# kcat/openal-soft

Measured on NVIDIA H100. Metric: voice-samples/s mixed (HRTF, bsinc24, 1024-frame updates), higher is better.
Workload: dtype f32

## Files before the change

openal-soft_b200/csrc/mixer_kernels.cuh:

```cuda
#pragma once
#include <cstdint>
#include <cuda_runtime.h>

#include "voice_structs.hpp"
#include "async_ptx.cuh"

namespace b200mix {

constexpr int kLine = 1024;
constexpr int kHrirLen = 128;
constexpr int kHist = 64;
constexpr int kEdge = 24;
constexpr int kPad = 48;
constexpr int kResBuf = kLine + 256 + kPad;
constexpr int kSrcSizeMax = kResBuf - kEdge;
constexpr int kAccumLen = kLine + kHrirLen;
constexpr float kSilence = 0.00001f;
constexpr float kEps = 1.1920929e-07f;

constexpr uint32_t kVfStatic = 1u<<2, kVfLooping = 1u<<3, kVfHrtf = 1u<<4;
constexpr uint32_t kVfFading = 1u<<8, kVfHaveBuffer = 1u<<9, kVfCoefDirty = 1u<<10;
constexpr uint32_t kUpNoBuffer = 1u<<11;
constexpr uint32_t kVfChannelMask = 0xffu<<16;

struct alignas(16) BufferRec {
    const void *data;
    uint32_t frames, type, channels, pad;
};

struct alignas(16) VoiceRec {
    uint32_t state;
    uint32_t flags;
    uint32_t buffer, resampler;
    int32_t  pos; uint32_t frac, step, loop_start;
    uint32_t loop_end; float bsinc_sf; uint32_t bsinc_m, bsinc_l;
    uint32_t bsinc_off, tgt_delay0, tgt_delay1; float tgt_gain;
    uint32_t old_delay0, old_delay1; float old_gain; uint32_t send_mask;
    uint32_t send_slot[kMaxSends]; uint32_t pad2[2];
    float prev[kPad];
    float hist[kHist];
};

struct VoiceResult { int32_t position; uint32_t position_frac, flags, buffers_done; };

struct alignas(16) FilterRec {
    float cur[2][5]; float tgt[2][5];
    float z[2][2];
    int32_t counter[2];
    uint32_t active;
    uint32_t pad[5];
};
static_assert(sizeof(FilterRec) == 128, "FilterRec layout");

struct MixParams {
    VoiceRec *voices; const BufferRec *buffers;
    float2 *hrtf_tgt; float2 *hrtf_old;
    float *dry_cur; float *dry_tgt;
    float *partial;
    VoiceResult *results;
    const float *bsinc_tab[3];
    const float *cubic_tab[2];
    uint32_t max_voices, frames, ir_pad, cd, num_sends;
    float *xscratch;
    uint32_t *sendinfo;
    const uint32_t *order;
    uint32_t num_order;
    FilterRec *filt;
    uint32_t filt_paths;
    const float *dline;
    uint4 *qhdr; const uint32_t *queue;
    uint32_t *claim;
};

constexpr uint32_t kMaxQueue = 32, kNoLoop = 0xffffffffu;

constexpr uint32_t kSiSend = 1u, kSiPlaying = 2u, kSiDeferred = 4u, kSiDirty = 8u, kSiDry = 16u,
    kSiHrtf = 32u;

__device__ __forceinline__ void group_sync(int id, int count)
{
    if(id == 1) asm volatile("bar.sync 1, %0;" :: "r"(count) : "memory");
    else asm volatile("bar.sync 2, %0;" :: "r"(count) : "memory");
}

__device__ __forceinline__ void prefetch_l2(const void *p)
{ asm volatile("prefetch.global.L2 [%0];" :: "l"(p)); }

__device__ __forceinline__ uint32_t sample_bytes(uint32_t type)
{ return type == 1u ? 2u : ((type == 0u || type >= 5u) ? 1u : (type == 4u ? 8u : 4u)); }

__device__ __forceinline__ void prefetch_span(const char *base, size_t bytes, size_t off,
    size_t len, int t, int gs)
{
    if(off >= bytes) return;
    if(off + len > bytes) len = bytes - off;
    const size_t first = off & ~size_t(127);
    for(size_t a = first + size_t(t)*128u;a < off + len;a += size_t(gs)*128u)
        prefetch_l2(base + a);
}

__device__ __forceinline__ float load_sample(const BufferRec &b, size_t idx)
{
    switch(b.type)
    {
    case 0: return (float(static_cast<const uint8_t*>(b.data)[idx]) - 128.0f) * (1.0f/128.0f);
    case 1: return float(static_cast<const int16_t*>(b.data)[idx]) * (1.0f/32768.0f);
    case 2: return float(static_cast<const int32_t*>(b.data)[idx]) * (1.0f/2147483648.0f);
    case 3: return static_cast<const float*>(b.data)[idx];
    case 4: return float(static_cast<const double*>(b.data)[idx]);
    }
    return 0.0f;
}

__device__ __forceinline__ void calc_buffer_size(uint32_t fracPos, uint32_t increment,
    uint32_t dstRemaining, uint32_t &dst, uint32_t &src)
{
    const uint32_t ext = increment <= 65536u;
    const uint64_t srcSize64 = ((uint64_t(dstRemaining - ext)*increment + fracPos) >> 16)
        + ext + kEdge;
    if(srcSize64 <= uint64_t(kSrcSizeMax)) { dst = dstRemaining; src = uint32_t(srcSize64); return; }
    const uint64_t dstSize64 = ((uint64_t(kSrcSizeMax - kEdge)<<16) - fracPos) / increment;
    if(dstSize64 < dstRemaining) { dst = uint32_t(dstSize64) & ~3u; src = kSrcSizeMax; return; }
    dst = dstRemaining; src = kSrcSizeMax;
}

__device__ __forceinline__ int32_t add_sat(int32_t a, int32_t b)
{
    long long r = (long long)a + b;
    r = r > 2147483647ll ? 2147483647ll : (r < -2147483648ll ? -2147483648ll : r);
    return int32_t(r);
}

__device__ __forceinline__ float to_float(uint8_t v) { return (float(v) - 128.0f) * (1.0f/128.0f); }
__device__ __forceinline__ float to_float(int16_t v) { return float(v) * (1.0f/32768.0f); }
__device__ __forceinline__ float to_float(int32_t v) { return float(v) * (1.0f/2147483648.0f); }
__device__ __forceinline__ float to_float(float v) { return v; }
__device__ __forceinline__ float to_float(double v) { return float(v); }
struct MulawByte { uint8_t v; };
struct AlawByte { uint8_t v; };
__device__ __forceinline__ float to_float(MulawByte b)
{
    const uint32_t u = (~uint32_t(b.v)) & 0xffu;
    const int s = int((((u & 0x0fu)<<3) + 0x84u) << ((u>>4)&7u)) - 0x84;
    return float((u & 0x80u) ? -s : s) * (1.0f/32768.0f);
}
__device__ __forceinline__ float to_float(AlawByte b)
{
    const uint32_t a = uint32_t(b.v) ^ 0x55u;
    const uint32_t e = (a>>4)&7u, m = a & 0x0fu;
    const int s = (e == 0u) ? int((m<<4) + 8u) : int(((m<<4) + 0x108u) << (e-1u));
    return float((a & 0x80u) ? s : -s) * (1.0f/32768.0f);
}

template<typename T> __device__ __forceinline__ T ld_raw(const T *p) { return __ldg(p); }
template<> __device__ __forceinline__ MulawByte ld_raw(const MulawByte *p)
{ return MulawByte{__ldg(reinterpret_cast<const uint8_t*>(p))}; }
template<> __device__ __forceinline__ AlawByte ld_raw(const AlawByte *p)
{ return AlawByte{__ldg(reinterpret_cast<const uint8_t*>(p))}; }

constexpr int kPackB = 688;
static_assert(kPackB >= (kResBuf + 8 + 1)/2 && kPackB + (kResBuf + 8 + 1)/2 <= kResBuf + 8 + 24
    && (kPackB % 32) == 16, "16-bit window copies must fit the float window's storage");

__device__ __forceinline__ float win_at(const float *win, bool packed, uint32_t k)
{
    if(!packed) return win[k];
    const uint16_t y = reinterpret_cast<const uint16_t*>(win)[k];
    return float(int(y) - 32768) * (1.0f/32768.0f);
}

struct FillArgs {
    float *dst; uint32_t count, uintPos, q0, firstRun, loopStart, loopSize, lastFrame, channels;
    bool looping, pastEnd, simpleWrap;
};

__device__ __forceinline__ void filter_clear(FilterRec &fr, int t)
{
    if(t < 10) fr.cur[t/5][t%5] = fr.tgt[t/5][t%5];
    else if(t < 14) fr.z[(t-10)>>1][(t-10)&1] = 0.0f;
    else if(t < 16) fr.counter[t-14] = 0;
}

template<typename T, int GS>
__device__ __forceinline__ void fill_window(const FillArgs &A, const T *__restrict__ src, int t)
{
    for(uint32_t k0 = t;k0 < A.count;k0 += 8u*GS)
    {
        T raw[8];
        #pragma unroll
        for(int u = 0;u < 8;++u)
        {
            uint32_t k = k0 + uint32_t(u)*GS;
            k = k < A.count ? k : A.count-1u;
            uint32_t q;
            if(!A.looping) q = min(A.uintPos + k, A.lastFrame);
            else if(k < A.firstRun) q = A.q0 + k;
            else if(A.simpleWrap) q = A.loopStart + (k - A.firstRun);
            else q = A.loopStart + (k - A.firstRun)%A.loopSize;
            raw[u] = ld_raw(src + size_t(q)*A.channels);
        }
        #pragma unroll
        for(int u = 0;u < 8;++u)
        {
            const uint32_t k = k0 + uint32_t(u)*GS;
            if(k < A.count) A.dst[k] = A.pastEnd ? 0.0f : to_float(raw[u]);
        }
    }
}

constexpr int kWinFloats = kResBuf + 8 + 24;
template<int CDR>
struct alignas(16) GroupSmem {
    static constexpr int kTabStride = kPad + 2;
    float win[kWinFloats];
    alignas(8) float tabF[32*kTabStride];
    alignas(8) float tabD[32*kTabStride];
    float x[CDR > 0 ? kLine : 1];
    float newGain[32];
    uint64_t tmaBar;
    uint32_t claimed;
};

template<int GS, int OPT, int FP>
struct alignas(16) FirSmem {
    static constexpr int kLLen = FP + OPT*GS;
    static constexpr int kOLen = FP + kHist + FP + 32;
    float2 lLR[kLLen];
    float2 oLR[kOLen];
    float x[kHist + kLine];
    float2 coefT[kHrirLen], coefO[kHrirLen];
};

__device__ __forceinline__ float2 fma2_rn(float2 a, float2 b, float2 c)
{ return make_float2(__fmaf_rn(a.x, b.x, c.x), __fmaf_rn(a.y, b.y, c.y)); }

template<int OPT, int FP>
__device__ __forceinline__ void fir_pass(float2 (&acc)[OPT], const float2 *__restrict__ in,
    const float2 *__restrict__ coef, int irpad, int t0)
{
    constexpr int JB = 8;
    for(int jb = 0;jb < irpad;jb += JB)
    {
        float2 w[OPT+JB-1];
        const float2 *p = in + FP + t0 - jb - (JB-1);
        #pragma unroll
        for(int k = 0;k < OPT+JB-1;++k) w[k] = p[k];
        #pragma unroll
        for(int jj = 0;jj < JB;++jj)
        {
            const float2 c = coef[jb+jj];
            #pragma unroll
            for(int r = 0;r < OPT;++r)
                acc[r] = fma2_rn(c, w[r - jj + (JB-1)], acc[r]);
        }
    }
}

__device__ __forceinline__ uint32_t claim_voice(const MixParams &P, uint32_t &slot, int t, int bar,
    int gs, uint32_t groups)
{
    group_sync(bar, gs);
    if(t == 0)
    {
        uint32_t oi = atomicAdd(P.claim, 1u);
        if(oi >= P.num_order && atomicAdd(P.claim + 1, 1u) == groups - 1u)
        {
            atomicExch(P.claim, 0u);
            atomicExch(P.claim + 1, 0u);
        }
        slot = oi;
    }
    group_sync(bar, gs);
    return slot;
}


__device__ __forceinline__ bool voice_early_out(const MixParams &P, VoiceRec &rec, uint32_t v,
    uint32_t vstate, uint4 h1, int t)
{
    if(vstate != 1u && vstate != 2u)
    {
        if(t == 0)
        {
            if(P.results) P.results[v] = VoiceResult{int32_t(h1.x), h1.y, 1u<<7, 0u};
            if(P.sendinfo) P.sendinfo[v] = 0u;
        }
        return true;
    }
    if(h1.z < 1u)
    {
        if(t == 0)
        {
            if(vstate == 2u) rec.state = 0u;
            if(P.sendinfo) P.sendinfo[v] = 0u;
            if(P.results)
                P.results[v] = VoiceResult{int32_t(h1.x), h1.y, (vstate == 2u) ? (1u<<7) : 1u, 0u};
        }
        return true;
    }
    return false;
}

template<int GS>
__device__ __forceinline__ void build_phase_table(const MixParams &P, float *tabF, float *tabD,
    uint32_t resampler, uint32_t increment, uint4 h2, uint4 h3, int t,
    uint32_t &m, uint32_t &tapOff, uint32_t &ms)
{
    m = 0; tapOff = 0; ms = 5;
    if(resampler >= 4u)
    {
        m = h2.z;
        tapOff = kEdge - h2.w;
        const float *tab = P.bsinc_tab[(resampler-4u)>>1] + h3.x;
        const bool full = (increment > 65536u) && (resampler & 1u);
        const float sf = __uint_as_float(h2.y);
        const uint32_t rowLen = 2u*m;
        const float *tab2 = tab + 64u*m;
        ms = m + 1u;
        for(uint32_t c = t;c < rowLen;c += GS)
        {
            float *dstc = (c < m) ? (tabF + c) : (tabD + (c - m));
            #pragma unroll 1
            for(uint32_t p0 = 0;p0 < 32u;p0 += 8u)
            {
                float a[8], b[8];
                #pragma unroll
                for(int u = 0;u < 8;++u)
                {
                    a[u] = __ldg(tab + (p0+u)*rowLen + c);
                    b[u] = full ? __ldg(tab2 + (p0+u)*rowLen + c) : 0.0f;
                }
                #pragma unroll
                for(int u = 0;u < 8;++u)
                    dstc[(p0+u)*ms] = full ? fmaf(sf, b[u], a[u]) : a[u];
            }
        }
    }
    else if(resampler >= 2u)
    {
        m = 4; tapOff = kEdge - 1; ms = 5;
        const float *tab = P.cubic_tab[resampler-2u];
        for(uint32_t e = t;e < 128u;e += GS)
        {
            const uint32_t pi = e>>2, j = e&3u;
            tabF[pi*ms + j] = tab[pi*8u + j];
            tabD[pi*ms + j] = tab[pi*8u + 4u + j];
        }
    }
}

template<int GS>
__device__ __forceinline__ void prefetch_next_voices(const MixParams &P, uint32_t oi, uint32_t groups,
    int t)
{
    const uint32_t o2 = oi + 2u*groups, o1 = oi + groups;
    const uint32_t v2 = o2 < P.num_order ? P.order[o2] : 0xffffffffu;
    const uint32_t v1 = o1 < P.num_order ? P.order[o1] : 0xffffffffu;
    if(v2 < P.max_voices && t < 5)
        prefetch_l2(reinterpret_cast<const char*>(&P.voices[v2]) + t*128);
    if(v1 < P.max_voices)
    {
        const VoiceRec &nx = P.voices[v1];
        if((nx.state == 1u || nx.state == 2u) && (nx.flags & kVfHaveBuffer) && nx.step >= 1u)
        {
            const BufferRec nb = P.buffers[nx.buffer];
            const size_t fb = size_t(sample_bytes(nb.type))*nb.channels;
            const size_t bytes = size_t(nb.frames)*fb;
            const uint32_t p0 = nx.pos < 0 ? 0u : uint32_t(nx.pos);
            const size_t need = size_t((uint64_t(P.frames)*nx.step + nx.frac) >> 16) + kPad;
            const char *base = static_cast<const char*>(nb.data);
            prefetch_span(base, bytes, size_t(p0)*fb, need*fb, t, GS);
            if((nx.flags & kVfLooping) && p0 + need > nx.loop_end && nx.loop_end > p0)
                prefetch_span(base, bytes, size_t(nx.loop_start)*fb,
                    (p0 + need - nx.loop_end)*fb, t, GS);
        }
    }
}

template<int GS>
__device__ __forceinline__ void hold_end_sample(float *srcBuffer, uint32_t srcn, int t, int bar)
{
    const uint32_t avail = srcn < uint32_t(kEdge) ? srcn : uint32_t(kEdge);
    const uint32_t tofill = srcn > uint32_t(kEdge) ? srcn : uint32_t(kEdge);
    uint32_t best = 0;
    for(uint32_t i = 1;i < avail;++i)
        if(fabsf(srcBuffer[i]) < fabsf(srcBuffer[best])) best = i;
    const float held = srcBuffer[best];
    group_sync(bar, GS);
    for(uint32_t k = best+1+t;k < tofill;k += GS) srcBuffer[k] = held;
}

template<int GS>
__device__ __forceinline__ bool stage_span_tma(float *win, uint64_t *tmaBar, uint32_t &tmaPhase,
    const BufferRec &buf, uint32_t flags, bool isQueue, bool looping, uint32_t loopStart,
    uint32_t loopEnd, uint32_t uintPos, uint32_t count, float *dst, int t, int bar)
{
    if(isQueue || buf.type != 1u || buf.channels != 1u || ((flags >> 16) & 0xffu) != 0u || count == 0u)
        return false;
    const uint32_t loopSize = looping ? (loopEnd - loopStart) : 1u;
    const uint32_t q0 = !looping ? uintPos : ((uintPos < loopEnd) ? uintPos
        : ((uintPos-loopStart)%loopSize + loopStart));
    const uint32_t run1 = looping ? min(count, loopEnd - q0) : count;
    const uint32_t run2 = count - run1;
    const bool fits = looping ? (run2 <= loopSize && loopEnd <= buf.frames)
                              : (uintPos + count <= buf.frames);
    if(!fits) return false;
    const int16_t *base = static_cast<const int16_t*>(buf.data);
    const uintptr_t a1 = reinterpret_cast<uintptr_t>(base + q0);
    const uintptr_t a2 = reinterpret_cast<uintptr_t>(base + loopStart);
    const uint32_t lead1 = uint32_t(a1 & 15u) >> 1, lead2 = uint32_t(a2 & 15u) >> 1;
    const uint32_t bytes1 = ((run1 + lead1)*2u + 15u) & ~15u;
    const uint32_t bytes2 = run2 ? (((run2 + lead2)*2u + 15u) & ~15u) : 0u;
    constexpr uint32_t kWinBytes = uint32_t(kWinFloats*sizeof(float));
    unsigned char *wbytes = reinterpret_cast<unsigned char*>(win);
    unsigned char *raw2 = wbytes + kWinBytes - bytes2;
    unsigned char *raw1 = raw2 - bytes1;
    if(t == 0)
    {
        fence_proxy_async_smem();
        mbar_expect_tx(tmaBar, bytes1 + bytes2);
        bulk_g2s(raw1, reinterpret_cast<const void*>(a1 & ~uintptr_t(15)), bytes1, tmaBar);
        if(run2)
            bulk_g2s(raw2, reinterpret_cast<const void*>(a2 & ~uintptr_t(15)), bytes2, tmaBar);
    }
    mbar_wait(tmaBar, tmaPhase);
    tmaPhase ^= 1u;
    const int16_t *r1 = reinterpret_cast<const int16_t*>(raw1) + lead1;
    const int16_t *r2 = reinterpret_cast<const int16_t*>(raw2) + lead2;
    constexpr int PERW = (kSrcSizeMax + GS - 1)/GS;
    float v[PERW];
    #pragma unroll
    for(int u = 0;u < PERW;++u)
    {
        const uint32_t k = uint32_t(t) + uint32_t(u)*GS;
        int16_t x = 0;
        if(k < count) x = k < run1 ? r1[k] : r2[k - run1];
        v[u] = to_float(x);
    }
    group_sync(bar, GS);
    #pragma unroll
    for(int u = 0;u < PERW;++u)
    {
        const uint32_t k = uint32_t(t) + uint32_t(u)*GS;
        if(k < count) dst[k] = v[u];
    }
    return true;
}

template<int GS>
__device__ __forceinline__ bool gather_span(const MixParams &P, const BufferRec &buf, uint32_t flags,
    bool isQueue, uint4 qh, const uint32_t *qitems, bool looping, uint32_t loopStart, uint32_t loopEnd,
    uint32_t uintPos, uint32_t count, float *dst, int t, int bar)
{
    uint32_t done = 0, item = qh.x ? qh.y : kNoLoop, qpos = uintPos;
    bool more = true, winInt = true;
    while(more)
    {
        BufferRec rb = buf;
        FillArgs fa;
        if(!isQueue)
        {
            const uint32_t loopSize = looping ? (loopEnd - loopStart) : 1u;
            const uint32_t q0 = !looping ? uintPos : ((uintPos < loopEnd) ? uintPos
                : ((uintPos-loopStart)%loopSize + loopStart));
            const uint32_t firstRun = looping ? (loopEnd - q0) : 0u;
            const uint32_t lastFrame = buf.frames ? buf.frames-1u : 0u;
            const bool pastEnd = !looping && !(buf.frames > uintPos);
            const bool simpleWrap = looping && count <= firstRun + loopSize;
            fa = FillArgs{dst, count, uintPos, q0, firstRun, loopStart, loopSize,
                lastFrame, buf.channels, looping, pastEnd, simpleWrap};
            done = count; more = false;
        }
        else
        {
            bool found = false;
            while(item != kNoLoop && done < count)
            {
                rb = P.buffers[qitems[item]];
                if(qpos >= rb.frames)
                {
                    qpos -= rb.frames;
                    item = (item + 1u < qh.x) ? item + 1u : qh.z;
                    continue;
                }
                found = true;
                break;
            }
            if(!found) break;
            const uint32_t run = min(count - done, rb.frames - qpos);
            fa = FillArgs{dst + done, run, qpos, qpos, 0u, 0u, 1u, rb.frames-1u,
                rb.channels, false, false, false};
            done += run; qpos = 0u;
            item = (item + 1u < qh.x) ? item + 1u : qh.z;
            more = done < count;
        }
        winInt = winInt && (rb.type <= 1u || rb.type >= 5u);
        const uint32_t ch = ((flags >> 16) & 0xffu) < rb.channels ? ((flags >> 16) & 0xffu) : 0u;
        switch(rb.type)
        {
        case 0: fill_window<uint8_t, GS>(fa, static_cast<const uint8_t*>(rb.data) + ch, t); break;
        case 1: fill_window<int16_t, GS>(fa, static_cast<const int16_t*>(rb.data) + ch, t); break;
        case 2: fill_window<int32_t, GS>(fa, static_cast<const int32_t*>(rb.data) + ch, t); break;
        case 3: fill_window<float, GS>(fa, static_cast<const float*>(rb.data) + ch, t); break;
        case 4: fill_window<double, GS>(fa, static_cast<const double*>(rb.data) + ch, t); break;
        case 5: fill_window<MulawByte, GS>(fa, static_cast<const MulawByte*>(rb.data) + ch, t); break;
        default: fill_window<AlawByte, GS>(fa, static_cast<const AlawByte*>(rb.data) + ch, t); break;
        }
    }
    if(done < count)
    {
        group_sync(bar, GS);
        const float held = done ? dst[done-1u] : 0.0f;
        for(uint32_t k = done + t;k < count;k += GS) dst[k] = held;
    }
    return winInt;
}

template<int GS>
__device__ __forceinline__ void pack_window16(float *win, uint32_t srcn, int t, int bar)
{
    constexpr int PER = (kResBuf + 8 + GS - 1)/GS;
    const uint32_t L = min(uint32_t(kEdge) + srcn + 8u, uint32_t(kResBuf + 8));
    float v[PER];
    #pragma unroll
    for(int u = 0;u < PER;++u)
    {
        const uint32_t k = uint32_t(t) + uint32_t(u)*GS;
        v[u] = k < L ? win[k] : 0.0f;
    }
    group_sync(bar, GS);
    uint16_t *pa = reinterpret_cast<uint16_t*>(win);
    uint16_t *pb = pa + 2*kPackB;
    #pragma unroll
    for(int u = 0;u < PER;++u)
    {
        const uint32_t k = uint32_t(t) + uint32_t(u)*GS;
        if(k < L)
        {
            const uint16_t y = uint16_t(__float2int_rn(v[u]*32768.0f) + 32768);
            pa[k] = y;
            if(k) pb[k-1u] = y;
        }
    }
    group_sync(bar, GS);
}

template<int GS>
__device__ __forceinline__ void resample_chunk(const float *win, const float *tabF, const float *tabD,
    float *xs, uint32_t loaded, uint32_t dstn, uint32_t increment, uint32_t fracPos,
    uint32_t resampler, uint32_t m, uint32_t tapOff, uint32_t ms, bool packedWin, int t)
{
    const float *srcBuffer = win + kEdge;
    if(increment == 65536u && fracPos == 0u)
    {
        for(uint32_t k = t;k < dstn;k += GS) xs[loaded+k] = srcBuffer[k];
    }
    else if(packedWin)
    {
        const uint32_t *wordsA = reinterpret_cast<const uint32_t*>(win);
        const uint32_t *wordsB = wordsA + kPackB;
        const float2 bias = make_float2(-8421376.0f, -8421376.0f);
        const float2 one = make_float2(1.0f, 1.0f);
        for(uint32_t k = t;k < dstn;k += 2u*GS)
        {
            const uint32_t kB = k + GS;
            const bool hasB = kB < dstn;
            const uint64_t fpA = uint64_t(k)*increment + fracPos;
            const uint64_t fpB = uint64_t(hasB ? kB : k)*increment + fracPos;
            const uint32_t fracA = uint32_t(fpA) & 0xffffu, fracB = uint32_t(fpB) & 0xffffu;
            const float pfA = float(fracA & 2047u) * (1.0f/2048.0f);
            const float pfB = float(fracB & 2047u) * (1.0f/2048.0f);
            const float *FA = tabF + (fracA>>11)*ms, *DA = tabD + (fracA>>11)*ms;
            const float *FB = tabF + (fracB>>11)*ms, *DB = tabD + (fracB>>11)*ms;
            const uint32_t posA = tapOff + uint32_t(fpA>>16), posB = tapOff + uint32_t(fpB>>16);
            const uint32_t *wA = ((posA & 1u) ? wordsB : wordsA) + (posA >> 1);
            const uint32_t *wB = ((posB & 1u) ? wordsB : wordsA) + (posB >> 1);
            const float2 pA = make_float2(pfA, pfA), pB = make_float2(pfB, pfB);
            float2 a0 = make_float2(0.0f, 0.0f), a1 = a0, b0 = a0, b1 = a0;
            for(uint32_t j = 0;j < m;j += 4)
            {
                const uint32_t wa0 = wA[(j>>1)], wa1 = wA[(j>>1)+1u];
                const uint32_t wb0 = wB[(j>>1)], wb1 = wB[(j>>1)+1u];
                const float2 sA0 = fma2_rn(make_float2(__uint_as_float(__byte_perm(wa0, 0x4B00u, 0x5410u)),
                    __uint_as_float(__byte_perm(wa0, 0x4B00u, 0x5432u))), one, bias);
                const float2 sA1 = fma2_rn(make_float2(__uint_as_float(__byte_perm(wa1, 0x4B00u, 0x5410u)),
                    __uint_as_float(__byte_perm(wa1, 0x4B00u, 0x5432u))), one, bias);
                const float2 sB0 = fma2_rn(make_float2(__uint_as_float(__byte_perm(wb0, 0x4B00u, 0x5410u)),
                    __uint_as_float(__byte_perm(wb0, 0x4B00u, 0x5432u))), one, bias);
                const float2 sB1 = fma2_rn(make_float2(__uint_as_float(__byte_perm(wb1, 0x4B00u, 0x5410u)),
                    __uint_as_float(__byte_perm(wb1, 0x4B00u, 0x5432u))), one, bias);
                const float2 cA0 = fma2_rn(pA, make_float2(DA[j+0], DA[j+1]), make_float2(FA[j+0], FA[j+1]));
                const float2 cB0 = fma2_rn(pB, make_float2(DB[j+0], DB[j+1]), make_float2(FB[j+0], FB[j+1]));
                const float2 cA1 = fma2_rn(pA, make_float2(DA[j+2], DA[j+3]), make_float2(FA[j+2], FA[j+3]));
                const float2 cB1 = fma2_rn(pB, make_float2(DB[j+2], DB[j+3]), make_float2(FB[j+2], FB[j+3]));
                a0 = fma2_rn(cA0, sA0, a0);
                b0 = fma2_rn(cB0, sB0, b0);
                a1 = fma2_rn(cA1, sA1, a1);
                b1 = fma2_rn(cB1, sB1, b1);
            }
            xs[loaded+k] = ((a0.x + a1.x) + (a0.y + a1.y)) * (1.0f/32768.0f);
            if(hasB) xs[loaded+kB] = ((b0.x + b1.x) + (b0.y + b1.y)) * (1.0f/32768.0f);
        }
    }
    else if(resampler >= 2u)
    {
        const float *vals = win + tapOff;
        for(uint32_t k = t;k < dstn;k += 2u*GS)
        {
            const uint32_t kB = k + GS;
            const bool hasB = kB < dstn;
            const uint64_t fpA = uint64_t(k)*increment + fracPos;
            const uint64_t fpB = uint64_t(hasB ? kB : k)*increment + fracPos;
            const uint32_t fracA = uint32_t(fpA) & 0xffffu, fracB = uint32_t(fpB) & 0xffffu;
            const float pfA = float(fracA & 2047u) * (1.0f/2048.0f);
            const float pfB = float(fracB & 2047u) * (1.0f/2048.0f);
            const float *FA = tabF + (fracA>>11)*ms, *DA = tabD + (fracA>>11)*ms;
            const float *FB = tabF + (fracB>>11)*ms, *DB = tabD + (fracB>>11)*ms;
            const float *svA = vals + uint32_t(fpA>>16), *svB = vals + uint32_t(fpB>>16);
            const float2 pA = make_float2(pfA, pfA), pB = make_float2(pfB, pfB);
            float2 a0 = make_float2(0.0f, 0.0f), a1 = a0, b0 = a0, b1 = a0;
            for(uint32_t j = 0;j < m;j += 4)
            {
                const float2 cA0 = fma2_rn(pA, make_float2(DA[j+0], DA[j+1]), make_float2(FA[j+0], FA[j+1]));
                const float2 cB0 = fma2_rn(pB, make_float2(DB[j+0], DB[j+1]), make_float2(FB[j+0], FB[j+1]));
                const float2 cA1 = fma2_rn(pA, make_float2(DA[j+2], DA[j+3]), make_float2(FA[j+2], FA[j+3]));
                const float2 cB1 = fma2_rn(pB, make_float2(DB[j+2], DB[j+3]), make_float2(FB[j+2], FB[j+3]));
                a0 = fma2_rn(cA0, make_float2(svA[j+0], svA[j+1]), a0);
                b0 = fma2_rn(cB0, make_float2(svB[j+0], svB[j+1]), b0);
                a1 = fma2_rn(cA1, make_float2(svA[j+2], svA[j+3]), a1);
                b1 = fma2_rn(cB1, make_float2(svB[j+2], svB[j+3]), b1);
            }
            xs[loaded+k] = (a0.x + a1.x) + (a0.y + a1.y);
            if(hasB) xs[loaded+kB] = (b0.x + b1.x) + (b0.y + b1.y);
        }
    }
    else
    {
        const float *vals = srcBuffer;
        for(uint32_t k = t;k < dstn;k += GS)
        {
            const uint64_t fp = uint64_t(k)*increment + fracPos;
            const uint32_t pos = uint32_t(fp>>16), frac = uint32_t(fp) & 0xffffu;
            if(resampler == 0u) xs[loaded+k] = vals[pos];
            else
            {
                const float a = vals[pos], b = vals[pos+1];
                xs[loaded+k] = a + (b-a)*(float(frac)*(1.0f/65536.0f));
            }
        }
    }
}

template<int GS>
__device__ __forceinline__ void advance_chunk(float *win, float *prev, bool packedWin, bool silent,
    bool playing, uint32_t n, uint32_t &loaded, uint32_t dstn, uint32_t increment, uint32_t &fracPos,
    int32_t &intPos, int t, int bar)
{
    const uint32_t loadEnd = loaded + dstn;
    if(!silent && playing && n > loaded && n <= loadEnd)
    {
        const uint32_t dstOffset = n - loaded;
        const uint32_t srcOffset = uint32_t((uint64_t(dstOffset)*increment + fracPos) >> 16);
        for(int k = t;k < kPad;k += GS) prev[k] = win_at(win, packedWin, srcOffset + uint32_t(k));
    }
    loaded = loadEnd;
    if(loaded < n)
    {
        fracPos += dstn*increment;
        const uint32_t srcOffset = fracPos >> 16;
        fracPos &= 0xffffu;
        if(silent) intPos = add_sat(intPos, int32_t(srcOffset));
        else
        {
            if(intPos < 0) intPos += int32_t(srcOffset);
            else intPos = add_sat(intPos, int32_t(srcOffset));
            float carry = 0.0f;
            if(t < kPad) carry = win_at(win, packedWin, srcOffset + uint32_t(t));
            float carry2 = 0.0f;
            if(GS < kPad && t + GS < kPad) carry2 = win_at(win, packedWin, srcOffset + uint32_t(t) + GS);
            group_sync(bar, GS);
            if(t < kPad) win[t] = carry;
            if(GS < kPad && t + GS < kPad) win[t + GS] = carry2;
        }
    }
}

template<int GS, int CDR>
__device__ __forceinline__ void park_voice(const MixParams &P, const float *xs, uint32_t v,
    uint32_t sendMask, bool defer, bool isHrtf, bool playing, bool dirty, uint32_t counter, int t)
{
    const uint32_t n = P.frames;
    const bool sends = P.num_sends && sendMask;
    const bool park = sends || defer || CDR == 0;
    if(CDR > 0 && park)
        for(uint32_t k = t;k < n;k += GS) P.xscratch[size_t(v)*kLine + k] = xs[k];
    if(t == 0)
        P.sendinfo[v] = park ? ((sends ? kSiSend : 0u)
            | (playing ? kSiPlaying : 0u) | (defer ? kSiDeferred : 0u) | (dirty ? kSiDirty : 0u)
            | ((CDR == 0 && !isHrtf) ? kSiDry : 0u) | (isHrtf ? kSiHrtf : 0u) | (counter << 8)) : 0u;
}

template<int GS, int CDR>
__device__ __forceinline__ void mix_dry(float (&accD)[CDR][kLine/GS], const float *xs, float *newGain,
    const float *cur, const float *tgt, uint32_t cd, uint32_t n, uint32_t counter, bool playing, int t)
{
    constexpr int SPT = kLine / GS;
    const float delta = counter ? 1.0f/float(counter) : 0.0f;
    const uint32_t fadeLen = counter < n ? counter : n;
    for(uint32_t c = 0;c < cd;++c)
    {
        const float cg = counter ? cur[c] : tgt[c];
        const float tg = playing ? tgt[c] : 0.0f;
        const float step = (tg - cg)*delta;
        const bool fade = fabsf(step) > kEps;
        const bool early = fade && fadeLen < counter;
        const float flat = (!early && fabsf(tg) > kSilence) ? tg : 0.0f;
        const uint32_t start = fade ? fadeLen : 0u;
        #pragma unroll
        for(int r = 0;r < SPT;++r)
        {
            const uint32_t i = t + r*GS;
            float gsel = 0.0f;
            if(i < n)
                gsel = (fade && i < fadeLen) ? (cg + step*float(i)) : (i >= start ? flat : 0.0f);
            const float x = xs[i < n ? i : 0];
            if(c < uint32_t(CDR))
            {
                #pragma unroll
                for(int cc = 0;cc < CDR;++cc)
                    if(cc == int(c)) accD[cc][r] = __fmaf_rn(x, gsel, accD[cc][r]);
            }
        }
        if(t == 0)
            newGain[c] = early ? (cg + step*float(fadeLen)) : tg;
    }
}

__device__ __forceinline__ void store_dry_gains(float *cur, const float *newGain, uint32_t cd, int t)
{
    if(t == 0)
        for(uint32_t c = 0;c < cd;++c) cur[c] = newGain[c];
}

__device__ __forceinline__ void write_back_voice(const MixParams &P, VoiceRec &rec, uint32_t v,
    uint4 h1, uint32_t flags, uint32_t vstate, uint32_t increment, bool haveBuffer, bool isQueue,
    uint4 qh, const uint32_t *qitems, bool looping, uint32_t loopStart, uint32_t loopEnd,
    uint32_t bufFrames)
{
    uint32_t newFlags = (flags | kVfFading) & ~kVfCoefDirty;
    uint32_t newState = vstate;
    uint32_t buffersDone = 0u;
    int32_t pos = int32_t(h1.x); uint32_t frac = h1.y;
    if(vstate == 2u) newState = 0u;
    else
    {
        frac += increment*P.frames;
        const uint32_t done = frac >> 16;
        pos = add_sat(pos, int32_t(done));
        frac &= 0xffffu;
        if(haveBuffer && pos > 0 && isQueue)
        {
            uint32_t item = qh.x ? qh.y : kNoLoop;
            while(item != kNoLoop)
            {
                const uint32_t len = P.buffers[qitems[item]].frames;
                if(len > uint32_t(pos)) break;
                pos -= int32_t(len);
                ++buffersDone;
                item = (item + 1u < qh.x) ? item + 1u : qh.z;
            }
            if(item == kNoLoop) { newFlags &= ~kVfHaveBuffer; newState = 2u; }
            else if(item != qh.y) P.qhdr[v].y = item;
        }
        else if(haveBuffer && pos > 0)
        {
            if(looping)
            {
                uint32_t up = uint32_t(pos);
                if(up >= loopEnd)
                    pos = int32_t((up-loopStart)%(loopEnd-loopStart) + loopStart);
            }
            else if(uint32_t(pos) >= bufFrames)
            {
                newFlags &= ~kVfHaveBuffer;
                newState = 2u;
            }
        }
        rec.pos = pos; rec.frac = frac;
    }
    rec.flags = newFlags;
    rec.state = newState;
    if(P.results)
        P.results[v] = VoiceResult{pos, frac,
            newState == 1u ? 1u : (newState == 2u ? 2u : (1u<<7)), buffersDone};
}

template<int GS, int GROUPS, int CDR>
__device__ __forceinline__ void store_partial_row(const float (&accD)[CDR][kLine/GS], unsigned char *smem,
    float *partial, int g, int t)
{
    constexpr int SPT = kLine / GS;
    const size_t row = blockIdx.x;
    __syncthreads();
    float *stage = reinterpret_cast<float*>(smem);
    float *pd = partial + row*(size_t(CDR)*kLine);
    if(GROUPS == 1)
    {
        #pragma unroll
        for(int c = 0;c < CDR;++c)
            #pragma unroll
            for(int r = 0;r < SPT;++r)
                pd[c*kLine + t + r*GS] = accD[c][r];
    }
    else
    {
        for(int gg = 0;gg < GROUPS;++gg)
        {
            if(g == gg)
            {
                #pragma unroll
                for(int c = 0;c < CDR;++c)
                    #pragma unroll
                    for(int r = 0;r < SPT;++r)
                    {
                        float *dst = stage + c*kLine + t + r*GS;
                        if(gg == 0) *dst = accD[c][r]; else *dst += accD[c][r];
                    }
            }
            __syncthreads();
        }
        for(int o = threadIdx.x;o < CDR*kLine;o += GS*GROUPS) pd[o] = stage[o];
    }
}

constexpr int kMixGS = 64, kMixGroups = 2;

template<int GS, int GROUPS, int CDR>
__global__ void __launch_bounds__(GS*GROUPS, GS*GROUPS != 128 ? 1 : (CDR == 0 ? 5 : 3))
k_mix_voices(const MixParams P)
{
    using Smem = GroupSmem<CDR>;
    static_assert(CDR == 0 || sizeof(Smem)*GROUPS >= size_t(CDR)*kLine*sizeof(float),
        "the partial row is staged in the groups' storage");
    extern __shared__ __align__(16) unsigned char smem_raw[];
    const int g = threadIdx.x / GS;
    const int t = threadIdx.x % GS;
    Smem &S = reinterpret_cast<Smem*>(smem_raw)[g];
    const int bar = 1 + g;
    constexpr int SPT = kLine / GS;

    float accD[CDR > 0 ? CDR : 1][SPT];
    #pragma unroll
    for(int c = 0;c < (CDR > 0 ? CDR : 1);++c)
        #pragma unroll
        for(int r = 0;r < SPT;++r) accD[c][r] = 0.0f;

    const uint32_t n = P.frames;
    if(t == 0) { mbar_init(&S.tmaBar, 1u); mbar_fence_init(); }
    uint32_t tmaPhase = 0u;
    group_sync(bar, GS);

    const uint32_t groups = gridDim.x*GROUPS;
    for(uint32_t oi = CDR > 0 ? blockIdx.x*GROUPS + g : claim_voice(P, S.claimed, t, bar, GS, groups);
        oi < P.num_order;
        oi = CDR > 0 ? oi + groups : claim_voice(P, S.claimed, t, bar, GS, groups))
    {
        const uint32_t v = P.order[oi];
        VoiceRec &rec = P.voices[v];
        const uint4 *hp = reinterpret_cast<const uint4*>(&rec);
        const uint4 h0 = hp[0], h1 = hp[1], h2 = hp[2], h3 = hp[3], h4 = hp[4];
        const uint32_t vstate = h0.x;
        if(voice_early_out(P, rec, v, vstate, h1, t)) continue;
        const uint32_t increment = h1.z;
        const uint32_t flags = h0.y;
        const bool haveBuffer = (flags & kVfHaveBuffer) != 0;
        const BufferRec buf = P.buffers[haveBuffer ? h0.z : 0u];
        const uint32_t loopStart = h1.w, loopEnd = h2.x;
        int32_t intPos = int32_t(h1.x);
        uint32_t fracPos = h1.y;
        bool looping = (flags & kVfLooping) != 0;
        if((flags & kVfStatic) && looping && haveBuffer && intPos >= 0
            && uint32_t(intPos) >= loopEnd)
            looping = false;
        const uint32_t resampler = h0.w;
        const bool isQueue = !(flags & kVfStatic) && P.qhdr != nullptr;
        const uint4 qh = isQueue ? P.qhdr[v] : make_uint4(0u, 0u, kNoLoop, 0u);
        const uint32_t *qitems = P.queue + size_t(v)*kMaxQueue;
        const bool isHrtf = CDR == 0 && P.ir_pad != 0u && (flags & kVfHrtf);
        const bool dirty = (flags & kVfCoefDirty) != 0;
        FilterRec *dfilt = P.filt ? P.filt + size_t(v)*P.filt_paths : nullptr;
        const bool defer = dfilt && dfilt->active;
        const bool playing = vstate == 1u;

        for(int k = t;k < kPad;k += GS) S.win[k] = rec.prev[k];
        uint32_t m, tapOff, ms;
        build_phase_table<GS>(P, S.tabF, S.tabD, resampler, increment, h2, h3, t, m, tapOff, ms);
        float *xs = CDR > 0 ? S.x : P.xscratch + size_t(v)*kLine;
        if(CDR == 0) prefetch_next_voices<GS>(P, oi, groups, t);

        for(uint32_t loaded = 0;loaded < n;)
        {
            uint32_t dstn, srcn;
            calc_buffer_size(fracPos, increment, n-loaded, dstn, srcn);
            uint32_t srcDelay = 0;
            bool silent = false;
            bool packedWin = false;
            if(dstn == 0u) { dstn = n - loaded; silent = true; }
            if(intPos < 0)
            {
                srcDelay = uint32_t(-intPos);
                if(srcDelay >= srcn) silent = true;
            }
            group_sync(bar, GS);
            if(silent)
            {
                for(uint32_t k = t;k < dstn;k += GS) xs[loaded+k] = 0.0f;
                for(uint32_t k = t;k < srcn;k += GS) S.win[kEdge+k] = 0.0f;
            }
            else
            {
                float *srcBuffer = S.win + kEdge;
                bool winInt = false;
                if(!haveBuffer) hold_end_sample<GS>(srcBuffer, srcn, t, bar);
                else
                {
                    const uint32_t uintPos = intPos < 0 ? 0u : uint32_t(intPos);
                    const uint32_t count = srcn - srcDelay;
                    float *dst = srcBuffer + srcDelay;
                    for(uint32_t k = t;k < srcDelay;k += GS) srcBuffer[k] = 0.0f;
                    winInt = stage_span_tma<GS>(S.win, &S.tmaBar, tmaPhase, buf, flags, isQueue, looping,
                            loopStart, loopEnd, uintPos, count, dst, t, bar)
                        || gather_span<GS>(P, buf, flags, isQueue, qh, qitems, looping, loopStart, loopEnd,
                            uintPos, count, dst, t, bar);
                }
                group_sync(bar, GS);

                packedWin = resampler >= 4u && winInt && !(increment == 65536u && fracPos == 0u);
                if(packedWin) pack_window16<GS>(S.win, srcn, t, bar);
                resample_chunk<GS>(S.win, S.tabF, S.tabD, xs, loaded, dstn, increment, fracPos,
                    resampler, m, tapOff, ms, packedWin, t);
            }
            advance_chunk<GS>(S.win, rec.prev, packedWin, silent, playing, n, loaded, dstn, increment,
                fracPos, intPos, t, bar);
        }
        group_sync(bar, GS);

        const uint32_t counter = (flags & kVfFading) ? (n < 64u ? n : 64u) : 0u;
        if(P.sendinfo)
            park_voice<GS, CDR>(P, xs, v, h4.w, defer, isHrtf, playing, dirty, counter, t);
        if(dfilt && !defer) filter_clear(*dfilt, t);
        if constexpr(CDR > 0)
            if(!defer)
                mix_dry<GS, CDR>(accD, xs, S.newGain, P.dry_cur + size_t(v)*P.cd, P.dry_tgt + size_t(v)*P.cd,
                    P.cd, n, counter, playing, t);
        if(t == 0)
            write_back_voice(P, rec, v, h1, flags, vstate, increment, haveBuffer, isQueue, qh, qitems,
                looping, loopStart, loopEnd, buf.frames);
        group_sync(bar, GS);
        if(CDR > 0 && !defer) store_dry_gains(P.dry_cur + size_t(v)*P.cd, S.newGain, P.cd, t);
        group_sync(bar, GS);
    }

    if constexpr(CDR > 0) store_partial_row<GS, GROUPS, CDR>(accD, smem_raw, P.partial, g, t);
}

template<int GROUPS, int CDR>
union DeferredSmem {
    struct { float x[kLine]; float newGain[32]; } group[GROUPS];
    float stage[CDR*kLine];
};

template<int GS, int GROUPS, int CDR>
__global__ void __launch_bounds__(GS*GROUPS)
k_mix_deferred(const MixParams P)
{
    extern __shared__ __align__(16) unsigned char smem_raw[];
    const int g = threadIdx.x / GS;
    const int t = threadIdx.x % GS;
    auto &S = reinterpret_cast<DeferredSmem<GROUPS, CDR>*>(smem_raw)->group[g];
    const int bar = 1 + g;
    constexpr int SPT = kLine / GS;

    float accD[CDR][SPT];
    #pragma unroll
    for(int c = 0;c < CDR;++c)
        #pragma unroll
        for(int r = 0;r < SPT;++r) accD[c][r] = 0.0f;

    const uint32_t n = P.frames;
    const uint32_t groups = gridDim.x*GROUPS;
    for(uint32_t oi = blockIdx.x*GROUPS + g;oi < P.num_order;oi += groups)
    {
        const uint32_t v = P.order[oi];
        const uint32_t info = P.sendinfo[v];
        if(!(info & kSiDeferred)) continue;
        const float *fl = P.dline + size_t(v)*kLine;
        for(uint32_t k = t;k < n;k += GS) S.x[k] = fl[k];
        group_sync(bar, GS);
        mix_dry<GS, CDR>(accD, S.x, S.newGain, P.dry_cur + size_t(v)*P.cd, P.dry_tgt + size_t(v)*P.cd,
            P.cd, n, (info >> 8) & 0xffu, (info & kSiPlaying) != 0, t);
        group_sync(bar, GS);
        store_dry_gains(P.dry_cur + size_t(v)*P.cd, S.newGain, P.cd, t);
    }

    store_partial_row<GS, GROUPS, CDR>(accD, smem_raw, P.partial, g, t);
}

constexpr int kFirGS = 64, kFirGroups = 2, kFirCtasPerSm = 4;

template<int OPT, int FP>
__global__ void __launch_bounds__(kFirGS*kFirGroups, kFirCtasPerSm)
k_hrtf_fir(const MixParams P)
{
    constexpr int GS = kFirGS, GROUPS = kFirGroups;
    using Smem = FirSmem<GS, OPT, FP>;
    extern __shared__ __align__(16) unsigned char smem_raw[];
    const int g = threadIdx.x / GS;
    const int t = threadIdx.x % GS;
    Smem &S = reinterpret_cast<Smem*>(smem_raw)[g];
    const int bar = 1 + g;
    const int t0 = OPT*t;
    const uint32_t n = P.frames;

    float2 acc[OPT];
    #pragma unroll
    for(int r = 0;r < OPT;++r) acc[r] = make_float2(0.0f, 0.0f);

    const uint32_t stride = gridDim.x*GROUPS;
    for(uint32_t oi = blockIdx.x*GROUPS + g;oi < P.num_order;oi += stride)
    {
        const uint32_t v = P.order[oi];
        const uint32_t info = P.sendinfo[v];
        if(!(info & kSiHrtf)) continue;
        VoiceRec &rec = P.voices[v];
        const uint4 *hp = reinterpret_cast<const uint4*>(&rec);
        const uint4 h3 = hp[3], h4 = hp[4];
        const bool playing = (info & kSiPlaying) != 0;
        const bool dirty = (info & kSiDirty) != 0;
        const uint32_t counter = (info >> 8) & 0xffu;

        const float *line = ((info & kSiDeferred) ? P.dline : P.xscratch) + size_t(v)*kLine;
        for(int k = t;k < kHist;k += GS) S.x[k] = rec.hist[k];
        for(uint32_t k = t;k < n;k += GS) S.x[kHist + k] = line[k];
        const float2 *ct = P.hrtf_tgt + size_t(v)*P.ir_pad;
        const float2 *co = P.hrtf_old + size_t(v)*P.ir_pad;
        for(int k = t;k < int(P.ir_pad);k += GS)
        {
            const float2 c = ct[k];
            S.coefT[k] = c;
            S.coefO[k] = dirty ? co[k] : c;
        }
        group_sync(bar, GS);


        if(playing)
            for(int k = t;k < kHist;k += GS) rec.hist[k] = S.x[n + k];
        uint32_t oD0 = h4.x, oD1 = h4.y;
        float oGain = __uint_as_float(h4.z);
        const uint32_t tD0 = h3.y, tD1 = h3.z;
        const float tgtGain = __uint_as_float(h3.w);
        if(!counter) { oD0 = tD0; oD1 = tD1; oGain = tgtGain; }
        const bool sameFilter = !counter || (!dirty && oD0 == tD0 && oD1 == tD1);
        const float targetGain = tgtGain * (playing ? 1.0f : 0.0f);
        const uint32_t fademix = counter;
        float blendNewStep = 0.0f, oldStep = 0.0f;
        bool oldOn = false, newOn = false;
        float gainA = oGain;
        if(fademix)
        {
            const float gain = targetGain;
            blendNewStep = gain / float(fademix);
            oldStep = oGain / float(fademix);
            oldOn = oGain > kSilence;
            newOn = blendNewStep*float(fademix) > kSilence;
            gainA = gain;
        }
        const uint32_t todo = n - fademix;
        const float step2 = todo ? (targetGain - gainA) / float(todo) : 0.0f;

        const float *hs = S.x;
        for(int i = t;i < Smem::kLLen;i += GS)
        {
            const int s = i - FP;
            float l = 0.0f, r = 0.0f;
            if(s >= 0 && s < int(n))
            {
                float gnew;
                if(uint32_t(s) < fademix)
                    gnew = (newOn && s >= 1) ? blendNewStep*float(s) : 0.0f;
                else
                    gnew = gainA + step2*float(uint32_t(s) - fademix);
                l = hs[kHist - tD0 + s] * gnew;
                r = hs[kHist - tD1 + s] * gnew;
                if(sameFilter && oldOn && uint32_t(s) < fademix)
                {
                    const float gold = oldStep*float(fademix - uint32_t(s));
                    l += hs[kHist - oD0 + s] * gold;
                    r += hs[kHist - oD1 + s] * gold;
                }
            }
            S.lLR[i] = make_float2(l, r);
        }
        const bool oldPass = !sameFilter && oldOn;
        if(oldPass)
            for(int i = t;i < Smem::kOLen;i += GS)
            {
                const int s = i - FP;
                float l = 0.0f, r = 0.0f;
                if(s >= 0 && uint32_t(s) < fademix)
                {
                    const float gold = oldStep*float(fademix - uint32_t(s));
                    l = hs[kHist - oD0 + s] * gold;
                    r = hs[kHist - oD1 + s] * gold;
                }
                S.oLR[i] = make_float2(l, r);
            }
        group_sync(bar, GS);

        {
            const uint32_t o2 = oi + 2u*stride, o1 = oi + stride;
            const uint32_t v2 = o2 < P.num_order ? P.order[o2] : 0xffffffffu;
            const uint32_t v1 = o1 < P.num_order ? P.order[o1] : 0xffffffffu;
            if(v2 < P.max_voices)
            {
                if(t < 5) prefetch_l2(reinterpret_cast<const char*>(&P.voices[v2]) + t*128);
                else if(t < 5 + int((P.ir_pad*8u + 127u)/128u))
                    prefetch_l2(reinterpret_cast<const char*>(P.hrtf_tgt + size_t(v2)*P.ir_pad) + (t-5)*128);
            }
            if(v1 < P.max_voices && t < int(kLine*sizeof(float)/128u))
            {
                const float *nl = ((P.sendinfo[v1] & kSiDeferred) ? P.dline : P.xscratch) + size_t(v1)*kLine;
                prefetch_l2(reinterpret_cast<const char*>(nl) + t*128);
            }
        }

        const int irpad = int(P.ir_pad);
        fir_pass<OPT, FP>(acc, S.lLR, S.coefT, irpad, t0);
        if(oldPass && t0 < int(kHist) + irpad)
            fir_pass<OPT, FP>(acc, S.oLR, S.coefO, irpad, t0);
        if(t == 0)
        {
            rec.old_delay0 = tD0; rec.old_delay1 = tD1;
            rec.old_gain = targetGain;
        }
        group_sync(bar, GS);
    }

    const size_t row = blockIdx.x;
    __syncthreads();
    float *stage = reinterpret_cast<float*>(smem_raw);
    for(int gg = 0;gg < GROUPS;++gg)
    {
        if(g == gg)
        {
            #pragma unroll
            for(int r = 0;r < OPT;++r)
            {
                const int o = t0 + r;
                if(o < kAccumLen)
                {
                    if(gg == 0) { stage[o] = acc[r].x; stage[kAccumLen + o] = acc[r].y; }
                    else { stage[o] += acc[r].x; stage[kAccumLen + o] += acc[r].y; }
                }
            }
            if(gg == 0 && GS*OPT < kAccumLen)
                for(int o = GS*OPT + t;o < kAccumLen;o += GS) { stage[o] = 0.0f; stage[kAccumLen + o] = 0.0f; }
        }
        __syncthreads();
    }
    float *pl = P.partial + row*(2*kAccumLen);
    for(int o = threadIdx.x;o < 2*kAccumLen;o += GS*GROUPS) pl[o] = stage[o];
}


constexpr int kReduceCols = 8, kReduceSegs = 128;
__global__ void __launch_bounds__(1024)
k_reduce_rows(const float *__restrict__ partial, uint32_t rows, uint32_t len,
    float *__restrict__ out, int accumulate)
{
    __shared__ float4 sm[kReduceSegs][kReduceCols];
    const uint32_t col = threadIdx.x & (kReduceCols-1), seg = threadIdx.x / kReduceCols;
    const uint32_t e4 = blockIdx.x*kReduceCols + col;
    float4 s = make_float4(0.f, 0.f, 0.f, 0.f);
    if(e4*4u < len)
    {
        const uint32_t per = (rows + kReduceSegs - 1u)/kReduceSegs;
        const uint32_t r0 = seg*per, r1 = (r0 + per < rows) ? r0 + per : rows;
        const float4 *p = reinterpret_cast<const float4*>(partial) + e4;
        const size_t stride4 = len/4u;
        uint32_t r = r0;
        for(;r + 4u <= r1;r += 4u)
        {
            const float4 a = __ldg(p + size_t(r)*stride4), b = __ldg(p + size_t(r+1)*stride4);
            const float4 c = __ldg(p + size_t(r+2)*stride4), d = __ldg(p + size_t(r+3)*stride4);
            s.x += a.x; s.y += a.y; s.z += a.z; s.w += a.w;
            s.x += b.x; s.y += b.y; s.z += b.z; s.w += b.w;
            s.x += c.x; s.y += c.y; s.z += c.z; s.w += c.w;
            s.x += d.x; s.y += d.y; s.z += d.z; s.w += d.w;
        }
        for(;r < r1;++r)
        {
            const float4 a = __ldg(p + size_t(r)*stride4);
            s.x += a.x; s.y += a.y; s.z += a.z; s.w += a.w;
        }
    }
    sm[seg][col] = s;
    __syncthreads();
    #pragma unroll
    for(uint32_t width = kReduceSegs/4u;width >= 1u;width /= 4u)
    {
        float4 tot = make_float4(0.f, 0.f, 0.f, 0.f);
        const bool on = seg < width;
        if(on)
        {
            tot = sm[seg*4u][col];
            #pragma unroll
            for(uint32_t k = 1;k < 4u;++k)
            {
                const float4 a = sm[seg*4u + k][col];
                tot.x += a.x; tot.y += a.y; tot.z += a.z; tot.w += a.w;
            }
        }
        __syncthreads();
        if(on) sm[seg][col] = tot;
        __syncthreads();
        if(width == 2u) break;
    }
    if(seg == 0 && e4*4u < len)
    {
        float4 tot = sm[0][col];
        const float4 b = sm[1][col];
        tot.x += b.x; tot.y += b.y; tot.z += b.z; tot.w += b.w;
        float4 *o = reinterpret_cast<float4*>(out) + e4;
        if(accumulate)
        {
            const float4 a = *o;
            tot.x += a.x; tot.y += a.y; tot.z += a.z; tot.w += a.w;
        }
        *o = tot;
    }
}

__global__ void __launch_bounds__(256)
k_reduce_few(const float *__restrict__ partial, uint32_t rows, uint32_t len,
    float *__restrict__ out, int accumulate)
{
    const uint32_t e4 = blockIdx.x*blockDim.x + threadIdx.x;
    if(e4*4u >= len) return;
    const float4 *p = reinterpret_cast<const float4*>(partial) + e4;
    const size_t stride4 = len/4u;
    float4 v[16];
    #pragma unroll
// ... 1069 lines not shown
```

Measured before the change: 28.83 billion.

## Pack TMA-staged int16 samples directly into resampler window and reuse FIR window registers

When the TMA-staged source span does not wrap around a loop, the int16 samples are now packed straight from the raw bulk-copy buffer into the paired 16-bit window layout the bsinc resampler uses. This skips the intermediate float conversion pass and the separate pack_window16 pass. The HRTF FIR inner loop now processes two coefficient blocks per iteration, shifting the register window instead of reloading all of it, which cuts shared-memory loads. The send mask is read from the record on demand instead of through an extra 16-byte header load, at the cost of more intricate shuffle and funnel-shift logic with edge cases.

Result: faster. 29.87 billion (median of 6 runs) (+3.6%).

```diff
diff --git a/openal-soft_b200/csrc/mixer_kernels.cuh b/openal-soft_b200/csrc/mixer_kernels.cuh
--- a/openal-soft_b200/csrc/mixer_kernels.cuh
+++ b/openal-soft_b200/csrc/mixer_kernels.cuh
@@ -239,16 +239,30 @@
     const float2 *__restrict__ coef, int irpad, int t0)
 {
     constexpr int JB = 8;
-    for(int jb = 0;jb < irpad;jb += JB)
-    {
-        float2 w[OPT+JB-1];
+    constexpr int W = OPT + JB - 1;
+    for(int jb = 0;jb < irpad;jb += 2*JB)
+    {
         const float2 *p = in + FP + t0 - jb - (JB-1);
+        float2 w[W];
         #pragma unroll
-        for(int k = 0;k < OPT+JB-1;++k) w[k] = p[k];
+        for(int k = 0;k < W;++k) w[k] = p[k];
         #pragma unroll
         for(int jj = 0;jj < JB;++jj)
         {
             const float2 c = coef[jb+jj];
+            #pragma unroll
+            for(int r = 0;r < OPT;++r)
+                acc[r] = fma2_rn(c, w[r - jj + (JB-1)], acc[r]);
+        }
+        if(jb + JB >= irpad) break;
+        #pragma unroll
+        for(int k = W-1;k >= JB;--k) w[k] = w[k-JB];
+        #pragma unroll
+        for(int k = 0;k < JB;++k) w[k] = p[k - JB];
+        #pragma unroll
+        for(int jj = 0;jj < JB;++jj)
+        {
+            const float2 c = coef[jb+JB+jj];
             #pragma unroll
             for(int r = 0;r < OPT;++r)
                 acc[r] = fma2_rn(c, w[r - jj + (JB-1)], acc[r]);
@@ -391,9 +405,64 @@
 }
 
 template<int GS>
+__device__ __forceinline__ void pack_span16(float *win, const unsigned char *raw, uint32_t lead,
+    uint32_t srcDelay, uint32_t count, int t, int bar)
+{
+    constexpr int NW = (kResBuf + 8 + 1)/2;
+    constexpr int PER = (NW + GS - 1)/GS;
+    static_assert((GS/32)*(32*PER - 1) >= NW + 1, "the warps' runs must cover every word");
+    const uint32_t lane = uint32_t(t) & 31u;
+    const uint32_t w0 = uint32_t(t >> 5)*(32u*PER - 1u) + lane;
+    const uint32_t lo = uint32_t(kEdge) + srcDelay;
+    const uint32_t nw = (min(lo + count + 8u, uint32_t(kResBuf + 8)) + 1u)/2u;
+    const uint32_t off = lo - lead;
+    const uint32_t *rw = reinterpret_cast<const uint32_t*>(raw) - int((off + 1u) >> 1);
+    const uint32_t sh = (off & 1u)*16u;
+    uint32_t wa[PER];
+    #pragma unroll
+    for(int u = 0;u < PER;++u)
+    {
+        const uint32_t w = w0 + uint32_t(u)*32u;
+        wa[u] = (w <= nw && 2u*w + 1u >= lo) ? rw[w] : 0u;
+    }
+    #pragma unroll
+    for(int u = 0;u < PER;++u)
+    {
+        const uint32_t w = w0 + uint32_t(u)*32u;
+        uint32_t r1 = __shfl_sync(0xffffffffu, (u + 1 < PER && lane == 0u) ? wa[u + 1 < PER ? u + 1 : u] : wa[u],
+            (lane + 1u) & 31u);
+        if(u + 1 == PER && lane == 31u && w <= nw && 2u*w + 3u >= lo) r1 = rw[w + 1u];
+        uint32_t a = __funnelshift_r(wa[u], r1, sh) ^ 0x80008000u;
+        const int d = int(lo) - int(2u*w);
+        const uint32_t m = (d >= 1 ? 0x0000ffffu : 0u) | (d >= 2 ? 0xffff0000u : 0u);
+        a = (a & ~m) | (0x80008000u & m);
+        if(u == 0 && w < uint32_t(kEdge/2))
+            a = uint32_t(uint16_t(__float2int_rn(win[2u*w]*32768.0f) + 32768))
+                | (uint32_t(uint16_t(__float2int_rn(win[2u*w + 1u]*32768.0f) + 32768)) << 16);
+        wa[u] = a;
+    }
+    group_sync(bar, GS);
+    uint32_t *pa = reinterpret_cast<uint32_t*>(win);
+    uint32_t *pb = pa + kPackB;
+    #pragma unroll
+    for(int u = 0;u < PER;++u)
+    {
+        const uint32_t w = w0 + uint32_t(u)*32u;
+        const uint32_t next = __shfl_sync(0xffffffffu, (u + 1 < PER && lane == 0u) ? wa[u + 1 < PER ? u + 1 : u] : wa[u],
+            (lane + 1u) & 31u);
+        if(w < nw)
+        {
+            if(u > 0 || lane > 0u || t < 32) pa[w] = wa[u];
+            if(u + 1 < PER || lane < 31u) pb[w] = __funnelshift_r(wa[u], next, 16u);
+        }
+    }
+}
+
+template<int GS>
 __device__ __forceinline__ bool stage_span_tma(float *win, uint64_t *tmaBar, uint32_t &tmaPhase,
     const BufferRec &buf, uint32_t flags, bool isQueue, bool looping, uint32_t loopStart,
-    uint32_t loopEnd, uint32_t uintPos, uint32_t count, float *dst, int t, int bar)
+    uint32_t loopEnd, uint32_t uintPos, uint32_t srcDelay, uint32_t count, bool pack, bool &packed,
+    int t, int bar)
 {
     if(isQueue || buf.type != 1u || buf.channels != 1u || ((flags >> 16) & 0xffu) != 0u || count == 0u)
         return false;
@@ -425,6 +494,13 @@
     }
     mbar_wait(tmaBar, tmaPhase);
     tmaPhase ^= 1u;
+    if(pack && !run2)
+    {
+        pack_span16<GS>(win, raw1, lead1, srcDelay, count, t, bar);
+        packed = true;
+        return true;
+    }
+    float *dst = win + kEdge + srcDelay;
     const int16_t *r1 = reinterpret_cast<const int16_t*>(raw1) + lead1;
     const int16_t *r2 = reinterpret_cast<const int16_t*>(raw2) + lead2;
     constexpr int PERW = (kSrcSizeMax + GS - 1)/GS;
@@ -868,7 +944,7 @@
         const uint32_t v = P.order[oi];
         VoiceRec &rec = P.voices[v];
         const uint4 *hp = reinterpret_cast<const uint4*>(&rec);
-        const uint4 h0 = hp[0], h1 = hp[1], h2 = hp[2], h3 = hp[3], h4 = hp[4];
+        const uint4 h0 = hp[0], h1 = hp[1], h2 = hp[2], h3 = hp[3];
         const uint32_t vstate = h0.x;
         if(voice_early_out(P, rec, v, vstate, h1, t)) continue;
         const uint32_t increment = h1.z;
@@ -921,22 +997,25 @@
             {
                 float *srcBuffer = S.win + kEdge;
                 bool winInt = false;
+                const bool pack = resampler >= 4u && !(increment == 65536u && fracPos == 0u);
                 if(!haveBuffer) hold_end_sample<GS>(srcBuffer, srcn, t, bar);
                 else
                 {
                     const uint32_t uintPos = intPos < 0 ? 0u : uint32_t(intPos);
                     const uint32_t count = srcn - srcDelay;
-                    float *dst = srcBuffer + srcDelay;
                     for(uint32_t k = t;k < srcDelay;k += GS) srcBuffer[k] = 0.0f;
                     winInt = stage_span_tma<GS>(S.win, &S.tmaBar, tmaPhase, buf, flags, isQueue, looping,
-                            loopStart, loopEnd, uintPos, count, dst, t, bar)
+                            loopStart, loopEnd, uintPos, srcDelay, count, pack, packedWin, t, bar)
                         || gather_span<GS>(P, buf, flags, isQueue, qh, qitems, looping, loopStart, loopEnd,
-                            uintPos, count, dst, t, bar);
+                            uintPos, count, srcBuffer + srcDelay, t, bar);
                 }
                 group_sync(bar, GS);
 
-                packedWin = resampler >= 4u && winInt && !(increment == 65536u && fracPos == 0u);
-                if(packedWin) pack_window16<GS>(S.win, srcn, t, bar);
+                if(pack && winInt && !packedWin)
+                {
+                    pack_window16<GS>(S.win, srcn, t, bar);
+                    packedWin = true;
+                }
                 resample_chunk<GS>(S.win, S.tabF, S.tabD, xs, loaded, dstn, increment, fracPos,
                     resampler, m, tapOff, ms, packedWin, t);
             }
@@ -947,7 +1026,7 @@
 
         const uint32_t counter = (flags & kVfFading) ? (n < 64u ? n : 64u) : 0u;
         if(P.sendinfo)
-            park_voice<GS, CDR>(P, xs, v, h4.w, defer, isHrtf, playing, dirty, counter, t);
+            park_voice<GS, CDR>(P, xs, v, rec.send_mask, defer, isHrtf, playing, dirty, counter, t);
         if(dfilt && !defer) filter_clear(*dfilt, t);
         if constexpr(CDR > 0)
             if(!defer)
```
